# a1q123456/image_stitching

Measured on AMD Instinct MI355X. Metric: 4K frames stitched/sec, higher is better.
Workload: dtype u8

## Files before the change

### image_stitching_amd/csrc/orb.hip

```cpp
#include "common.h"
#include "dev_math.h"
#include <algorithm>
#include <cmath>
#include <mutex>
#include <unordered_map>

#define ORB_MAX_LEVELS 16
#define ORB_BORDER 32

namespace {

struct LevelDesc {
    int w, h;
    int pp;
    int sp;
    size_t pad_off;
    size_t map_off;
    float scale;
    int nfeat;
    int n2;
    int tiles_x, tiles_y, tile_off;
    int cap1, cand_off;
    int cap2, fin_off;
    int tab_off;
};

struct Levels {
    int n;
    int fast_t, patch, half_patch, edge;
    LevelDesc d[ORB_MAX_LEVELS];
};

struct Work {
    uint8_t *pad, *blur, *score, *nms;
    int* hist;
    int* thr;
    int* tile_cnt;
    uint32_t* surv_xy;
    uint8_t* surv_sc;
    int* cnt1;
    int* cnt2;
    int* flags;
    uint32_t* cand_xy;
    float* cand_resp;
    uint32_t* fin_xy;
    float* fin_resp;
    int* tab;
    int* umax;
    int8_t* pattern;
};

constexpr int ORB_BATCH = 16;
struct OrbIO {
    const uint8_t* src[ORB_BATCH];
    size_t sstride[ORB_BATCH];
    int aligned[ORB_BATCH];
    MisKeyPoint* kps[ORB_BATCH];
    uint32_t* lxy[ORB_BATCH];
    int* n_dev[ORB_BATCH];
    uint8_t* desc[ORB_BATCH];
};
#define WS_OFF(p, f, ws) p = (decltype(p))((const char*)(p) + (size_t)(f) * (ws))

constexpr int GRAY_ROWS = 4;
__global__ __launch_bounds__(256) void gray_kernel(OrbIO io, int w, int h, uint8_t* dst, int pp, size_t ws) {
    const int x = (blockIdx.x * 256 + threadIdx.x) * 4, y0 = blockIdx.y * GRAY_ROWS, f = blockIdx.z;
    if (x >= w) return;
    const uint8_t* bgr = io.src[f];
    const size_t stride = io.sstride[f];
    const int aligned = io.aligned[f];
    WS_OFF(dst, f, ws);
    const int nrows = min(GRAY_ROWS, h - y0);
    if (aligned && x + 4 <= w) {
        unsigned w0[GRAY_ROWS], w1[GRAY_ROWS], w2[GRAY_ROWS];
#pragma unroll
        for (int r = 0; r < GRAY_ROWS; r++) {
            const unsigned* sp = reinterpret_cast<const unsigned*>(bgr + (size_t)min(y0 + r, h - 1) * stride + 3 * (size_t)x);
            w0[r] = sp[0]; w1[r] = sp[1]; w2[r] = sp[2];
        }
#pragma unroll
        for (int r = 0; r < GRAY_ROWS; r++) {
            if (r >= nrows) break;
            const unsigned g0 = ((w0[r] & 255) * 3735 + ((w0[r] >> 8) & 255) * 19235 + ((w0[r] >> 16) & 255) * 9798 + (1 << 14)) >> 15;
            const unsigned g1 = ((w0[r] >> 24) * 3735 + (w1[r] & 255) * 19235 + ((w1[r] >> 8) & 255) * 9798 + (1 << 14)) >> 15;
            const unsigned g2 = (((w1[r] >> 16) & 255) * 3735 + (w1[r] >> 24) * 19235 + (w2[r] & 255) * 9798 + (1 << 14)) >> 15;
            const unsigned g3 = (((w2[r] >> 8) & 255) * 3735 + ((w2[r] >> 16) & 255) * 19235 + (w2[r] >> 24) * 9798 + (1 << 14)) >> 15;
            *reinterpret_cast<unsigned*>(dst + (size_t)(y0 + r + ORB_BORDER) * pp + ORB_BORDER + x) = g0 | (g1 << 8) | (g2 << 16) | (g3 << 24);
        }
    } else {
        for (int r = 0; r < nrows; r++) {
            const uint8_t* s = bgr + (size_t)(y0 + r) * stride + 3 * (size_t)x;
            uint8_t* o = dst + (size_t)(y0 + r + ORB_BORDER) * pp + ORB_BORDER + x;
            for (int k = 0; k < 4 && x + k < w; k++) o[k] = (uint8_t)((s[3 * k] * 3735 + s[3 * k + 1] * 19235 + s[3 * k + 2] * 9798 + (1 << 14)) >> 15);
        }
    }
}

__device__ __forceinline__ unsigned byte_at(unsigned w0, unsigned w1, unsigned w2, int o) {
    const unsigned long long lo = (unsigned long long)w0 | ((unsigned long long)w1 << 32);
    return (o < 8 ? (unsigned)(lo >> (8 * o)) : (w2 >> (8 * (o - 8)))) & 255u;
}
#ifndef MIS_RS_ROWS
#define MIS_RS_ROWS 4
#endif
constexpr int RS_ROWS = MIS_RS_ROWS;
__global__ __launch_bounds__(256) void resize_kernel(const uint8_t* __restrict__ src, int sw, int sh, int spp, uint8_t* __restrict__ dst, int dw, int dh, int dpp,
                                                     const int* __restrict__ tab, size_t ws) {
    const int x = (blockIdx.x * 64 + (threadIdx.x & 63)) * 4;
    const int ybase = __builtin_amdgcn_readfirstlane((blockIdx.y * 4 + (threadIdx.x >> 6)) * RS_ROWS);
    if (x >= dw || ybase >= dh) return;
    WS_OFF(src, blockIdx.z, ws); WS_OFF(dst, blockIdx.z, ws);
    const int dw4 = (dw + 3) & ~3;
    const int *xo = tab, *xm = tab + dw4, *yo = tab + 2 * dw4, *ym = tab + 2 * dw4 + dh;
    const int4 o4 = *reinterpret_cast<const int4*>(xo + x), m4 = *reinterpret_cast<const int4*>(xm + x);
    const int xs[4] = {o4.x, o4.y, o4.z, o4.w}, ms[4] = {m4.x, m4.y, m4.z, m4.w};
    const int nvalid = min(4, dw - x), nrows = min(RS_ROWS, dh - ybase);
    const int base = xs[0] & ~3, last = xs[nvalid - 1] + 1 - base;
    const uint8_t* r0[RS_ROWS];
    const uint8_t* r1[RS_ROWS];
    int my1[RS_ROWS];
#pragma unroll
    for (int r = 0; r < RS_ROWS; r++) {
        const int y = min(ybase + r, dh - 1);
        const int y0 = yo[y], y1 = y0 + 1 < sh ? y0 + 1 : y0;
        my1[r] = ym[y];
        r0[r] = src + (size_t)(y0 + ORB_BORDER) * spp + ORB_BORDER;
        r1[r] = src + (size_t)(y1 + ORB_BORDER) * spp + ORB_BORDER;
    }
    uint8_t* out = dst + (size_t)(ybase + ORB_BORDER) * dpp + ORB_BORDER + x;
    unsigned res[RS_ROWS];
    if (last <= 11) {
        unsigned a[RS_ROWS][3], b[RS_ROWS][3];
#pragma unroll
        for (int r = 0; r < RS_ROWS; r++) {
            const unsigned* p0 = reinterpret_cast<const unsigned*>(r0[r] + base);
            const unsigned* p1 = reinterpret_cast<const unsigned*>(r1[r] + base);
            a[r][0] = p0[0]; a[r][1] = p0[1]; a[r][2] = p0[2]; b[r][0] = p1[0]; b[r][1] = p1[1]; b[r][2] = p1[2];
        }
#pragma unroll
        for (int r = 0; r < RS_ROWS; r++) res[r] = 0;
#pragma unroll
        for (int k = 0; k < 4; k++) {
            const int o = xs[k] - base, mx1 = ms[k], mx0 = 256 - mx1;
            const bool ok = k < nvalid;
            const int oo = ok ? o : 0;
            const bool p1 = oo >= 4, p2 = oo >= 8;
#pragma unroll
            for (int r = 0; r < RS_ROWS; r++) {
                const unsigned alo = p2 ? a[r][2] : (p1 ? a[r][1] : a[r][0]), ahi = p2 ? 0u : (p1 ? a[r][2] : a[r][1]);
                const unsigned blo = p2 ? b[r][2] : (p1 ? b[r][1] : b[r][0]), bhi = p2 ? 0u : (p1 ? b[r][2] : b[r][1]);
                const unsigned ta = __builtin_amdgcn_alignbyte(ahi, alo, (unsigned)oo & 3u), tb = __builtin_amdgcn_alignbyte(bhi, blo, (unsigned)oo & 3u);
                const unsigned h0 = (ta & 255u) * mx0 + ((ta >> 8) & 255u) * mx1;
                const unsigned h1 = (tb & 255u) * mx0 + ((tb >> 8) & 255u) * mx1;
                res[r] |= ok ? ((h0 * (256 - my1[r]) + h1 * my1[r] + (1u << 15)) >> 16) << (8 * k) : 0u;
            }
        }
    } else {
#pragma unroll
        for (int r = 0; r < RS_ROWS; r++) {
            res[r] = 0;
#pragma unroll
            for (int k = 0; k < 4; k++) {
                if (k >= nvalid) break;
                const int x0 = xs[k], x1 = x0 + 1 < sw ? x0 + 1 : x0, mx1 = ms[k], mx0 = 256 - mx1;
                const unsigned h0 = (unsigned)r0[r][x0] * mx0 + (unsigned)r0[r][x1] * mx1;
                const unsigned h1 = (unsigned)r1[r][x0] * mx0 + (unsigned)r1[r][x1] * mx1;
                res[r] |= ((h0 * (256 - my1[r]) + h1 * my1[r] + (1u << 15)) >> 16) << (8 * k);
            }
        }
    }
#pragma unroll
    for (int r = 0; r < RS_ROWS; r++) {
        if (r >= nrows) break;
        uint8_t* o = out + (size_t)r * dpp;
        if (nvalid == 4) *reinterpret_cast<unsigned*>(o) = res[r];
        else
            for (int k = 0; k < nvalid; k++) o[k] = (uint8_t)(res[r] >> (8 * k));
    }
}

template <bool SIDES>
__global__ __launch_bounds__(256) void border_kernel(Levels L, uint8_t* pad, size_t ws) {
    const int f = blockIdx.z / L.n;
    const LevelDesc& d = L.d[blockIdx.z - f * L.n];
    WS_OFF(pad, f, ws);
    const int B = ORB_BORDER, pw = d.w + 2 * B, ph = d.h + 2 * B;
    uint8_t* p = pad + d.pad_off;
    if (!SIDES) {
        const int px4 = (blockIdx.x * 256 + threadIdx.x) * 4;
        if (px4 >= pw) return;
        const bool inner = px4 >= B && px4 + 3 < B + d.w;
        unsigned v[4];
        size_t drow[4], srow[4];
#pragma unroll
        for (int r = 0; r < 4; r++) {
            const int yy = blockIdx.y * 4 + r, py = yy < B ? yy : ph - 2 * B + yy;
            srow[r] = (size_t)(mis_reflect101(py - B, d.h) + B) * d.pp; drow[r] = (size_t)py * d.pp;
        }
        if (inner) {
#pragma unroll
            for (int r = 0; r < 4; r++) v[r] = *reinterpret_cast<const unsigned*>(p + srow[r] + px4);
#pragma unroll
            for (int r = 0; r < 4; r++) *reinterpret_cast<unsigned*>(p + drow[r] + px4) = v[r];
        } else {
#pragma unroll
            for (int r = 0; r < 4; r++)
                for (int k = 0; k < 4 && px4 + k < pw; k++) p[drow[r] + px4 + k] = p[srow[r] + mis_reflect101(px4 + k - B, d.w) + B];
        }
        return;
    }
    const int t = blockIdx.x * 256 + threadIdx.x, row = t >> 4, g = t & 15;
    if (row >= d.h) return;
    const int px = g < 8 ? 4 * g : pw - B + 4 * (g - 8);
    const size_t ro = (size_t)(row + B) * d.pp;
    unsigned v = 0;
#pragma unroll
    for (int k = 0; k < 4; k++) v |= (unsigned)p[ro + mis_reflect101(px + k - B, d.w) + B] << (8 * k);
    if ((px & 3) == 0) *reinterpret_cast<unsigned*>(p + ro + px) = v;
    else
#pragma unroll
        for (int k = 0; k < 4; k++) p[ro + px + k] = (uint8_t)(v >> (8 * k));
}

__device__ __forceinline__ bool fast_pretest(const uint8_t* p, int pp, int t) {
    const int v = p[0], hi = v + t, lo = v - t;
    const int c0 = p[3 * pp], c4 = p[3], c8 = p[-3 * pp], c12 = p[-3];
    unsigned br = (c0 > hi) | ((c4 > hi) << 2) | ((c8 > hi) << 4) | ((c12 > hi) << 6);
    unsigned dk = (c0 < lo) | ((c4 < lo) << 2) | ((c8 < lo) << 4) | ((c12 < lo) << 6);
    const unsigned adj_b = br & ((br >> 2) | (br << 6)), adj_d = dk & ((dk >> 2) | (dk << 6));
    if (!((adj_b | adj_d) & 0x55)) return false;
    const int c2 = p[2 * pp + 2], c6 = p[-2 * pp + 2], c10 = p[-2 * pp - 2], c14 = p[2 * pp - 2];
    br |= ((c2 > hi) << 1) | ((c6 > hi) << 3) | ((c10 > hi) << 5) | ((c14 > hi) << 7);
    dk |= ((c2 < lo) << 1) | ((c6 < lo) << 3) | ((c10 < lo) << 5) | ((c14 < lo) << 7);
    const unsigned b2 = br | (br << 8), d2 = dk | (dk << 8);
    const unsigned rb = b2 & (b2 >> 1) & (b2 >> 2) & (b2 >> 3), rd = d2 & (d2 >> 1) & (d2 >> 2) & (d2 >> 3);
    return ((rb | rd) & 0xff) != 0;
}
__device__ __forceinline__ int fast_score_full(const uint8_t* p, int pp, int t) {
    const int v = p[0];
    int d[16];
    d[0] = v - p[3 * pp]; d[1] = v - p[3 * pp + 1]; d[2] = v - p[2 * pp + 2]; d[3] = v - p[pp + 3];
    d[4] = v - p[3]; d[5] = v - p[-pp + 3]; d[6] = v - p[-2 * pp + 2]; d[7] = v - p[-3 * pp + 1];
    d[8] = v - p[-3 * pp]; d[9] = v - p[-3 * pp - 1]; d[10] = v - p[-2 * pp - 2]; d[11] = v - p[-pp - 3];
    d[12] = v - p[-3]; d[13] = v - p[pp - 3]; d[14] = v - p[2 * pp - 2]; d[15] = v - p[3 * pp - 1];
    int n3[16], x3[16];
#pragma unroll
    for (int i = 0; i < 16; i++) {
        n3[i] = min(min(d[i], d[(i + 1) & 15]), d[(i + 2) & 15]);
        x3[i] = max(max(d[i], d[(i + 1) & 15]), d[(i + 2) & 15]);
    }
    int A = -512, Bm = 512;
#pragma unroll
    for (int i = 0; i < 16; i++) {
        A = max(A, min(min(n3[i], n3[(i + 3) & 15]), n3[(i + 6) & 15]));
        Bm = min(Bm, max(max(x3[i], x3[(i + 3) & 15]), x3[(i + 6) & 15]));
    }
    const int best = max(A, -Bm);
    return best > t ? best - 1 : 0;
}
__device__ __forceinline__ int fast_score_px(const uint8_t* p, int pp, int t) { return fast_pretest(p, pp, t) ? fast_score_full(p, pp, t) : 0; }

#ifndef MIS_FT_ROWS
#define MIS_FT_ROWS 64
#endif
constexpr int FT_COLS = 64, FT_ROWS = MIS_FT_ROWS, FG_PITCH = 96, FG_COL0 = 15, HIST_COPIES = 8;
constexpr int FT_WR = (FT_ROWS + 2 + 3) / 4;
constexpr int FT_SLOTS = FT_COLS * FT_ROWS / 4;
#ifdef MIS_ORB_STATS
__device__ unsigned long long g_orb_stats[8];
#endif
__global__ __launch_bounds__(256) void fast_nms_kernel(Levels L, const uint8_t* pad, int* hist, int* tile_cnt, uint32_t* surv_xy, uint8_t* surv_sc, size_t ws) {
    __shared__ __attribute__((aligned(16))) uint8_t g[(FT_ROWS + 10) * FG_PITCH];
    __shared__ __attribute__((aligned(16))) uint8_t sc[(FT_ROWS + 2) * (FT_COLS + 4)];
    __shared__ int lh[256];
    __shared__ int lcount;
    __shared__ uint32_t lxy[FT_SLOTS];
    __shared__ uint8_t lsc[FT_SLOTS];
    __shared__ unsigned short queue[(FT_ROWS + 2) * (FT_COLS + 2)];
    __shared__ int qcount;
    const int fz = blockIdx.z / L.n, lz = blockIdx.z - fz * L.n;
    const LevelDesc& d = L.d[lz];
    const int x0 = blockIdx.x * FT_COLS, y0 = blockIdx.y * FT_ROWS, t = threadIdx.x;
    if (x0 >= d.w || y0 >= d.h) return;
    WS_OFF(pad, fz, ws); WS_OFF(hist, fz, ws); WS_OFF(tile_cnt, fz, ws); WS_OFF(surv_xy, fz, ws); WS_OFF(surv_sc, fz, ws);
    lh[t] = 0;
    if (t == 0) { lcount = 0; qcount = 0; }
    {
        const int ph = d.h + 2 * ORB_BORDER;
        const uint8_t* src = pad + d.pad_off;
        const int px0 = x0 - 16 + ORB_BORDER, py0 = y0 - 4 + ORB_BORDER;
        for (int i = t; i < (FT_ROWS + 8) * (FG_PITCH / 16); i += 256) {
            const int r = i / (FG_PITCH / 16), c = i - r * (FG_PITCH / 16);
            const int py = min(py0 + r, ph - 1);
            int px = px0 + 16 * c;
            if (px + 15 >= d.pp) px = d.pp - 16;
            reinterpret_cast<uint4*>(g)[i] = *reinterpret_cast<const uint4*>(src + (size_t)py * d.pp + px);
        }
    }
    __syncthreads();
    const int SP = FT_COLS + 4;
    for (int i = t; i < (FT_ROWS + 2) * SP / 4; i += 256) reinterpret_cast<unsigned*>(sc)[i] = 0u;
    {
        const int wv = __builtin_amdgcn_readfirstlane(t >> 6), lane = t & 63;
        const unsigned ft = (unsigned)L.fast_t;
        const int r0 = FT_WR * wv;
        bool pass[FT_WR + 1];
        unsigned long long ball[FT_WR + 1];
        int total = 0;
        {
            const uint8_t* colp = g + r0 * FG_PITCH + (lane + FG_COL0);
            unsigned col[FT_WR + 6];
#pragma unroll
            for (int j = 0; j < FT_WR + 6; j++) col[j] = colp[j * FG_PITCH];
            const int x = x0 - 1 + lane;
            const bool xin = x >= 3 && x < d.w - 3;
            const uint8_t* rowp = g + (r0 + 3) * FG_PITCH + (lane + FG_COL0 - 3);
#pragma unroll
            for (int k = 0; k < FT_WR; k++) {
                const int r = r0 + k, y = y0 - 1 + r;
                const bool rowok = r < FT_ROWS + 2 && y >= 3 && y < d.h - 3;
                const unsigned v = col[k + 3];
                const unsigned dv = max(__builtin_amdgcn_sad_u8(col[k + 6], v, 0u), __builtin_amdgcn_sad_u8(col[k], v, 0u));
                const unsigned dh = max(__builtin_amdgcn_sad_u8(rowp[k * FG_PITCH + 6], v, 0u), __builtin_amdgcn_sad_u8(rowp[k * FG_PITCH], v, 0u));
                pass[k] = rowok & xin & (min(dv, dh) > ft);
                ball[k] = __ballot(pass[k]);
                total += __popcll(ball[k]);
            }
        }
        {
            const int k = lane >> 1, cc = FT_COLS + (lane & 1), r = r0 + k, y = y0 - 1 + r, x = x0 - 1 + cc;
            bool ps = false;
            if (lane < 2 * FT_WR && r < FT_ROWS + 2) {
                const uint8_t* pp = g + (r + 3) * FG_PITCH + (cc + FG_COL0);
                const unsigned v = pp[0];
                const unsigned dv = max(__builtin_amdgcn_sad_u8(pp[3 * FG_PITCH], v, 0u), __builtin_amdgcn_sad_u8(pp[-3 * FG_PITCH], v, 0u));
                const unsigned dh = max(__builtin_amdgcn_sad_u8(pp[3], v, 0u), __builtin_amdgcn_sad_u8(pp[-3], v, 0u));
                ps = x >= 3 && x < d.w - 3 && y >= 3 && y < d.h - 3 && min(dv, dh) > ft;
            }
            pass[FT_WR] = ps;
            ball[FT_WR] = __ballot(ps);
            total += __popcll(ball[FT_WR]);
        }
        int base = 0;
        if (lane == 0 && total) base = atomicAdd(&qcount, total);
        base = __builtin_amdgcn_readfirstlane(base);
        const unsigned long long below = (1ull << lane) - 1ull;
#pragma unroll
        for (int k = 0; k < FT_WR + 1; k++) {
            if (pass[k]) {
                const int r = k < FT_WR ? r0 + k : r0 + (lane >> 1), c = k < FT_WR ? lane : FT_COLS + (lane & 1);
                queue[base + __popcll(ball[k] & below)] = (unsigned short)(r * (FT_COLS + 2) + c);
            }
            base += __popcll(ball[k]);
        }
    }
    __syncthreads();
    for (int q = t; q < qcount; q += 256) {
        const int i = queue[q], r = i / (FT_COLS + 2), c = i - r * (FT_COLS + 2);
        const int fsv = fast_score_full(g + (r + 3) * FG_PITCH + (c + FG_COL0), FG_PITCH, L.fast_t);
        sc[r * SP + c] = (uint8_t)fsv;
#ifdef MIS_ORB_STATS
        if (fsv) atomicAdd(&g_orb_stats[3], 1ull);
#endif
    }
    __syncthreads();
    {
        const int nq = qcount;
        for (int q0 = 0; q0 < nq; q0 += 256) {
            const int q = q0 + t;
            bool keep = false;
// ... 280 lines not shown
        for (int k = 0; k < ORB_MAX_LEVELS; k++) c[k] = k < L.n ? cnt2[min(k, L.n - 1)] : 0;
#pragma unroll
        for (int k = 0; k < ORB_MAX_LEVELS; k++) {
            if (j >= total + c[k]) { base = total + c[k]; l = k + 1; }
            total += c[k];
        }
    }
    if (blockIdx.x == 0 && threadIdx.x == 0) *n_out = min(total, cap_out);
    if (j >= total || j >= cap_out) return;
    const LevelDesc& d = L.d[l];
    const int i = j - base;
    uint32_t xy = fin_xy[d.fin_off + i];
    int x = xy & 0xffff, y = xy >> 16;
    const int pp = d.pp, hp = L.half_patch;
    const uint8_t* ctr = pad + d.pad_off + (size_t)(y + ORB_BORDER) * pp + (x + ORB_BORDER);
    int m01 = 0, m10 = 0;
    const int u = lane - hp;
    if (with_angle && lane <= 2 * hp) {
        m10 = u * ctr[u];
        if (hp <= 15) {
            int um[16], vp[16], vm[16];
#pragma unroll
            for (int v = 1; v <= 15; ++v) um[v] = umax[min(v, hp)];
#pragma unroll
            for (int v = 1; v <= 15; ++v) { const int vv = min(v, hp); vp[v] = ctr[u + vv * pp]; vm[v] = ctr[u - vv * pp]; }
#pragma unroll
            for (int v = 1; v <= 15; ++v) {
                const bool in = v <= hp && abs(u) <= um[v];
                m10 += in ? u * (vp[v] + vm[v]) : 0;
                m01 += in ? v * (vp[v] - vm[v]) : 0;
            }
        } else {
            for (int v = 1; v <= hp; ++v) {
                if (abs(u) <= umax[v]) {
                    int vp = ctr[u + v * pp], vm = ctr[u - v * pp];
                    m10 += u * (vp + vm);
                    m01 += v * (vp - vm);
                }
            }
        }
    }
#pragma unroll
    for (int o = 32; o > 0; o >>= 1) { m01 += __shfl_xor(m01, o); m10 += __shfl_xor(m10, o); }
    if (lane == 0) {
        MisKeyPoint kp;
        kp.x = (float)x * d.scale; kp.y = (float)y * d.scale;
        kp.size = (float)L.patch * d.scale;
        kp.angle = with_angle ? mis_fast_atan2((float)m01, (float)m10) : 0.f;
        kp.response = fin_resp[d.fin_off + i];
        kp.octave = l;
        kps[base + i] = kp;
        kp_lxy[base + i] = xy;
    }
}

__global__ __launch_bounds__(256) void blur_kernel(Levels L, const uint8_t* pad, uint8_t* blur) {
    constexpr int TR = 32, TP = 80;
    __shared__ __attribute__((aligned(16))) uint8_t tile[(TR + 6) * TP];
    __shared__ __attribute__((aligned(16))) uint16_t hbuf[(TR + 6) * 64];
    const LevelDesc& d = L.d[blockIdx.z];
    const int pw = d.w + 2 * ORB_BORDER, ph = d.h + 2 * ORB_BORDER;
    const int tx0 = blockIdx.x * 64, ty0 = blockIdx.y * TR, t = threadIdx.x;
    if (tx0 >= pw || ty0 >= ph) return;
    const uint8_t* src = pad + d.pad_off;
    uint8_t* dst = blur + d.pad_off;
    for (int i = t; i < (TR + 6) * (TP / 4); i += 256) {
        const int r = i / (TP / 4), c = i - r * (TP / 4);
        const int sy = min(max(ty0 + r - 3, 0), ph - 1);
        int sx = tx0 - 4 + 4 * c;
        sx = min(max(sx, 0), d.pp - 4);
        reinterpret_cast<unsigned*>(tile)[i] = *reinterpret_cast<const unsigned*>(src + (size_t)sy * d.pp + sx);
    }
    __syncthreads();
    const int kq[7] = {18, 34, 48, 56, 48, 34, 18};
    for (int i = t; i < (TR + 6) * 16; i += 256) {
        const int r = i >> 4, cg = i & 15;
        const unsigned* p = reinterpret_cast<const unsigned*>(tile + r * TP + 4 * cg);
        const unsigned w0 = p[0], w1 = p[1], w2 = p[2];
        int b[12];
#pragma unroll
        for (int k = 0; k < 4; k++) { b[k] = (w0 >> (8 * k)) & 255; b[4 + k] = (w1 >> (8 * k)) & 255; b[8 + k] = (w2 >> (8 * k)) & 255; }
        unsigned short o[4];
#pragma unroll
        for (int k = 0; k < 4; k++) {
            int acc = 0;
#pragma unroll
            for (int j = 0; j < 7; j++) acc += kq[j] * b[k + 1 + j];
            o[k] = (unsigned short)acc;
        }
        *reinterpret_cast<uint2*>(hbuf + r * 64 + 4 * cg) = make_uint2(o[0] | ((unsigned)o[1] << 16), o[2] | ((unsigned)o[3] << 16));
    }
    __syncthreads();
    const int c = t & 63, px = tx0 + c;
    if (px >= pw) return;
    const int r0 = (t >> 6) * (TR / 4);
    int hv[TR / 4 + 6];
#pragma unroll
    for (int j = 0; j < TR / 4 + 6; j++) hv[j] = hbuf[(r0 + j) * 64 + c];
#pragma unroll
    for (int k = 0; k < TR / 4; k++) {
        const int r = r0 + k, py = ty0 + r;
        if (py >= ph) break;
        const int x = px - ORB_BORDER, y = py - ORB_BORDER;
        uint8_t o;
        if ((unsigned)x < (unsigned)d.w && (unsigned)y < (unsigned)d.h) {
            int acc = 0;
#pragma unroll
            for (int j = 0; j < 7; j++) acc += kq[j] * hv[k + j];
            o = (uint8_t)((acc + (1 << 15)) >> 16);
        } else o = tile[(r + 3) * TP + c + 4];
        dst[(size_t)py * d.pp + px] = o;
    }
}

__global__ __launch_bounds__(256) void describe_kernel(Levels L, const uint8_t* blur, const MisKeyPoint* kps, const uint32_t* kp_lxy,
                                                       const int* n_ptr, const int8_t* pattern, uint8_t* desc) {
    const int i = blockIdx.x * 8 + (threadIdx.x >> 5), b = threadIdx.x & 31;
    if (i >= *n_ptr) return;
    const MisKeyPoint kp = kps[i];
    const LevelDesc& d = L.d[kp.octave];
    const float inv = 1.f / d.scale;
    const int cx = mis_round_f(kp.x * inv), cy = mis_round_f(kp.y * inv);
    float ang = kp.angle * (float)(3.14159265358979323846 / 180.f);
    float sa, ca;
    mis_sincosf(ang, &sa, &ca);
    const int pp = d.pp;
    const uint8_t* ctr = blur + d.pad_off + (size_t)(cy + ORB_BORDER) * pp + (cx + ORB_BORDER);
    const int8_t* pat = pattern + b * 32;
    int val = 0;
#pragma unroll
    for (int bit = 0; bit < 8; bit++) {
        float x0 = (float)pat[4 * bit], y0 = (float)pat[4 * bit + 1], x1 = (float)pat[4 * bit + 2], y1 = (float)pat[4 * bit + 3];
        int ix0 = mis_round_f(x0 * ca - y0 * sa), iy0 = mis_round_f(x0 * sa + y0 * ca);
        int ix1 = mis_round_f(x1 * ca - y1 * sa), iy1 = mis_round_f(x1 * sa + y1 * ca);
        int t0 = ctr[iy0 * pp + ix0], t1 = ctr[iy1 * pp + ix1];
        val |= (t0 < t1) << bit;
    }
    desc[(size_t)i * 32 + b] = (uint8_t)val;
}

constexpr int DD_R = 28, DD_P = DD_R + 3, DD_N = 2 * DD_P + 1, DD_ROW_DW = (DD_N + 3 + 3) / 4, DD_PITCH = 4 * DD_ROW_DW + 4;
struct UMax16 { int v[16]; };
__global__ __launch_bounds__(256) void describe_direct_kernel(Levels L, const uint8_t* pad, OrbIO io, const int8_t* pattern, const int* umax, UMax16 um16, size_t ws) {
    __shared__ __attribute__((aligned(16))) uint8_t patch[4][DD_N * DD_PITCH];
    const int wave = threadIdx.x >> 6, lane = threadIdx.x & 63;
    const int i = blockIdx.x * 4 + wave, fr = blockIdx.y;
    WS_OFF(pad, fr, ws);
    MisKeyPoint* kps = io.kps[fr];
    const uint32_t* kp_lxy = io.lxy[fr];
    const int* n_ptr = io.n_dev[fr];
    uint8_t* desc = io.desc[fr];
    if (i >= *n_ptr) return;
    const MisKeyPoint kp = kps[i];
    const LevelDesc& d = L.d[kp.octave];
    const float inv = 1.f / d.scale;
    const int cx = mis_round_f(kp.x * inv), cy = mis_round_f(kp.y * inv);
    const int pp = d.pp;
    const uint8_t* org = pad + d.pad_off + (size_t)(cy + ORB_BORDER - DD_P) * pp + (cx + ORB_BORDER - DD_P);
    const int shift = (int)((uintptr_t)org & 3);
    const uint8_t* abase = org - shift;
    uint8_t* P = patch[wave];
    for (int k = lane; k < DD_N * DD_ROW_DW; k += 64) {
        const int r = k / DD_ROW_DW, c = k - r * DD_ROW_DW;
        reinterpret_cast<unsigned*>(P + r * DD_PITCH)[c] = *reinterpret_cast<const unsigned*>(abase + (size_t)r * pp + 4 * c);
    }
    __builtin_amdgcn_fence(__ATOMIC_ACQ_REL, "wavefront");
    __builtin_amdgcn_wave_barrier();
    const int c0 = DD_P * DD_PITCH + DD_P + shift;
    float kp_angle;
    {
        const int hp = L.half_patch;
        const uint8_t* ctr = P + c0;
        int m01 = 0, m10 = 0;
        const int u = lane - hp;
        if (lane <= 2 * hp) {
            m10 = u * ctr[u];
            if (hp <= 15) {
#pragma unroll 3
                for (int v = 1; v <= hp; ++v) {
                    const int vp = ctr[u + v * DD_PITCH], vm = ctr[u - v * DD_PITCH];
                    const bool in = abs(u) <= um16.v[v];
                    m10 += in ? u * (vp + vm) : 0;
                    m01 += in ? v * (vp - vm) : 0;
                }
            } else {
                for (int v = 1; v <= hp; ++v) {
                    if (abs(u) <= umax[v]) {
                        const int vp = ctr[u + v * DD_PITCH], vm = ctr[u - v * DD_PITCH];
                        m10 += u * (vp + vm);
                        m01 += v * (vp - vm);
                    }
                }
            }
        }
#pragma unroll
        for (int o = 32; o > 0; o >>= 1) { m01 += __shfl_xor(m01, o); m10 += __shfl_xor(m10, o); }
        kp_angle = mis_fast_atan2((float)m01, (float)m10);
        if (lane == 0) kps[i].angle = kp_angle;
    }
    float ang = kp_angle * (float)(3.14159265358979323846 / 180.f);
    float sa, ca;
    mis_sincosf(ang, &sa, &ca);
    const int b = lane & 31, h = lane >> 5;
    const int8_t* pat = pattern + b * 32 + h * 16;
    const unsigned* P32 = reinterpret_cast<const unsigned*>(P);
    auto blurred = [&](int ix, int iy) {
        const int a = c0 + (iy - 3) * DD_PITCH + (ix - 3);
        const bool inside = (unsigned)(cx + ix) < (unsigned)d.w && (unsigned)(cy + iy) < (unsigned)d.h;
        const unsigned* q = P32 + (a >> 2);
        const unsigned sh = (unsigned)(a & 3) << 3;
        const int kq[7] = {18, 34, 48, 56, 48, 34, 18};
        unsigned acc = 0, centre = 0;
#pragma unroll
        for (int j = 0; j < 7; j++) {
            const unsigned d0 = q[j * (DD_PITCH / 4)], d1 = q[j * (DD_PITCH / 4) + 1], d2 = q[j * (DD_PITCH / 4) + 2];
            const unsigned lo = __builtin_amdgcn_alignbit(d1, d0, sh), hi = __builtin_amdgcn_alignbit(d2, d1, sh);
            const unsigned hs = __builtin_amdgcn_udot4(lo, 0x38302212u, __builtin_amdgcn_udot4(hi, 0x00122230u, 0u, false), false);
            acc += (unsigned)kq[j] * hs;
            if (j == 3) centre = lo >> 24;
        }
        return inside ? (int)((acc + (1u << 15)) >> 16) : (int)centre;
    };
    int val = 0;
#ifndef DD_UNROLL
#define DD_UNROLL 1
#endif
#pragma unroll DD_UNROLL
    for (int bit = 0; bit < 4; bit++) {
        float x0 = (float)pat[4 * bit], y0 = (float)pat[4 * bit + 1], x1 = (float)pat[4 * bit + 2], y1 = (float)pat[4 * bit + 3];
        int ix0 = mis_round_f(x0 * ca - y0 * sa), iy0 = mis_round_f(x0 * sa + y0 * ca);
        int ix1 = mis_round_f(x1 * ca - y1 * sa), iy1 = mis_round_f(x1 * sa + y1 * ca);
        const int t0 = blurred(ix0, iy0), t1 = blurred(ix1, iy1);
        val |= (t0 < t1) << (bit + 4 * h);
    }
    val |= __shfl_xor(val, 32);
    if (h == 0) desc[(size_t)i * 32 + b] = (uint8_t)val;
}

constexpr int ORB_GATHER_MAX = 96;
struct GatherPtrs { const int* p[ORB_GATHER_MAX]; };
__global__ void gather_ints_kernel(GatherPtrs g, int n, int* __restrict__ out) {
    const int i = blockIdx.x * blockDim.x + threadIdx.x;
    if (i < n) out[i] = *g.p[i];
}

}

struct MisOrb {
    MisContext* ctx = nullptr;
    void (*enqueued_cb)(void*) = nullptr;
    void* enqueued_user = nullptr;
    MisOrbParams p;
    int max_w = 0, max_h = 0;
    int cur_w = 0, cur_h = 0;
    Levels L;
    Work w;
    size_t ws_stride = 0;
    int ws_frames = 0;
    int umax_host[64] = {0};
    int8_t pattern_host[1024] = {0};
    void* mem = nullptr;
    size_t pad_bytes = 0, map_bytes = 0;
    int cand_total = 0, fin_total = 0, tab_total = 0, surv_total = 0, out_cap = 0;
    std::vector<int> tab_host;
    int* host_counts = nullptr;
    bool direct_describe = false;
};

namespace {

void linear_exact_coeffs(int dlen, int slen, int* ofs, int* m1) {
    double inv = (double)dlen / (double)slen, scale = 1.0 / inv;
    for (int i = 0; i < dlen; i++) {
        double v = ((double)i + 0.5) * scale - 0.5;
        int iv = (int)floor(v);
        if (iv < 0) { ofs[i] = 0; m1[i] = 0; }
        else if (iv >= slen - 1) { ofs[i] = slen - 1; m1[i] = 0; }
        else { ofs[i] = iv; m1[i] = (int)lrint((v - (double)iv) * 256.0); }
    }
}

constexpr int ORB_MAX_LEVEL_FEATURES = 2048 - 128;

inline float level_scale(const MisOrbParams& p, int l) { return (float)pow((double)p.scale_factor, (double)l); }
inline int level_dim(int len, float sc) { return (int)lrint((double)((float)len / sc)); }

void level_budgets(const MisOrbParams& p, int* nfeat) {
    float factor = (float)(1.0 / (double)p.scale_factor);
    float nd = (float)p.nfeatures * (1 - factor) / (1 - (float)pow((double)factor, (double)p.nlevels));
    int sum = 0;
    for (int l = 0; l < p.nlevels - 1; l++) { nfeat[l] = (int)lrintf(nd); sum += nfeat[l]; nd *= factor; }
    nfeat[p.nlevels - 1] = std::max(p.nfeatures - sum, 0);
}

int check_level_sizes(MisContext* ctx, const MisOrbParams& p, int w, int h) {
    for (int l = 0; l < p.nlevels; l++) {
        const float sc = level_scale(p, l);
        MIS_CHECK(ctx, level_dim(w, sc) >= 1 && level_dim(h, sc) >= 1, MIS_E_UNSUPPORTED,
                  "ORB level %d of a %dx%d frame is empty (scale_factor %g, nlevels %d)", l, w, h, (double)p.scale_factor, p.nlevels);
    }
    return MIS_OK;
}

void plan_levels(MisOrb* o, int w, int h) {
    Levels& L = o->L;
    const MisOrbParams& p = o->p;
    L.n = p.nlevels; L.fast_t = p.fast_threshold; L.patch = p.patch_size; L.half_patch = p.patch_size / 2; L.edge = p.edge_threshold;
    size_t pad_off = 0, map_off = 0;
    int cand_off = 0, fin_off = 0, tab_off = 0, surv_off = 0;
    int nfeat[ORB_MAX_LEVELS];
    level_budgets(p, nfeat);
    for (int l = 0; l < L.n; l++) {
        LevelDesc& d = L.d[l];
        float sc = level_scale(p, l);
        d.scale = sc;
        d.w = level_dim(w, sc);
        d.h = level_dim(h, sc);
        d.pp = (int)mis_align_up((size_t)d.w + 2 * ORB_BORDER, 64);
        d.sp = (int)mis_align_up((size_t)d.w, 64);
        d.pad_off = pad_off; pad_off += (size_t)d.pp * (d.h + 2 * ORB_BORDER);
        d.map_off = map_off; map_off += (size_t)d.sp * d.h;
        d.nfeat = nfeat[l];
        d.n2 = p.score_type == 0 ? 2 * d.nfeat : d.nfeat;
        d.tiles_x = (d.w + FT_COLS - 1) / FT_COLS; d.tiles_y = (d.h + FT_ROWS - 1) / FT_ROWS;
        d.tile_off = surv_off; surv_off += d.tiles_x * d.tiles_y;
        d.cap1 = 4 * d.n2 + 4096;
        d.cap2 = std::min(d.nfeat + 128, 2048);
        d.cand_off = cand_off; cand_off += d.cap1;
        d.fin_off = fin_off; fin_off += d.cap2;
        d.tab_off = tab_off; tab_off += (2 * ((d.w + 3) & ~3) + 2 * d.h + 3) & ~3;
    }
    o->pad_bytes = pad_off; o->map_bytes = map_off; o->cand_total = cand_off; o->fin_total = fin_off; o->tab_total = tab_off; o->surv_total = surv_off;
    o->tab_host.assign(tab_off, 0);
    for (int l = 1; l < L.n; l++) {
        int* t = o->tab_host.data() + L.d[l].tab_off;
        const int dw4 = (L.d[l].w + 3) & ~3;
        linear_exact_coeffs(L.d[l].w, L.d[l - 1].w, t, t + dw4);
        linear_exact_coeffs(L.d[l].h, L.d[l - 1].h, t + 2 * dw4, t + 2 * dw4 + L.d[l].h);
    }
}

int upload_tables(MisOrb* o) {
    MisContext* ctx = o->ctx;
    if (o->tab_total)
        MIS_HIP(ctx, hipMemcpyAsync(o->w.tab, o->tab_host.data(), sizeof(int) * o->tab_total, hipMemcpyHostToDevice, ctx->stream));
    MIS_HIP(ctx, hipStreamSynchronize(ctx->stream));
    return MIS_OK;
}

std::mutex g_feat_mutex;
std::unordered_map<void*, size_t> g_feat_sizes;

int alloc_features(MisContext* ctx, int cap, int desc_cols, int desc_dtype, MisFeatures* f) {
    size_t kb = mis_align_up(sizeof(MisKeyPoint) * (size_t)cap, 256), db = mis_align_up((size_t)cap * desc_cols * mis_dtype_size(desc_dtype), 256);
    size_t lb = mis_align_up(sizeof(uint32_t) * (size_t)cap, 256);
    void* mem = nullptr;
    size_t got = 0;
    int rc = mis_pool_alloc(ctx, kb + db + lb + 256, &mem, &got);
    if (rc != MIS_OK) return rc;
    f->keypoints = (MisKeyPoint*)mem;
    f->descriptors = (uint8_t*)mem + kb;
    f->desc_cols = desc_cols; f->desc_dtype = desc_dtype;
    f->owner_ = mem;
    f->n = 0;
    std::lock_guard<std::mutex> lock(g_feat_mutex);
    g_feat_sizes[mem] = got;
    return MIS_OK;
}

inline uint32_t* feat_lxy(const MisFeatures* f, int cap) {
    size_t kb = mis_align_up(sizeof(MisKeyPoint) * (size_t)cap, 256), db = mis_align_up((size_t)cap * f->desc_cols * mis_dtype_size(f->desc_dtype), 256);
    return (uint32_t*)((uint8_t*)f->owner_ + kb + db);
}
inline int* feat_count(const MisFeatures* f, int cap) {
    size_t kb = mis_align_up(sizeof(MisKeyPoint) * (size_t)cap, 256), db = mis_align_up((size_t)cap * f->desc_cols * mis_dtype_size(f->desc_dtype), 256);
    size_t lb = mis_align_up(sizeof(uint32_t) * (size_t)cap, 256);
    return (int*)((uint8_t*)f->owner_ + kb + db + lb);
}

int enqueue_detect_group(MisOrb* o, const DevView* img, int w, int h, MisFeatures* out, int ng) {
    MisContext* ctx = o->ctx;
    const Levels& L = o->L;
// ... 373 lines not shown
```

Before: 3463.

## Use udot2/perm in resize, cheaper reflect in border, preload ORB pattern

Rewrites the bilinear resize fast path to pack pixel pairs with byte permutes and compute weights with udot2 dot products, replacing per-pixel selects and multiplies. Adds a single-fold reflect101 for border padding when the level is larger than the border. Loads the ORB pattern as one vector load, hoisted before the patch copy, and makes the octave index wave-uniform. Together these cut ALU work in several ORB kernels. The resize fast path now applies only when the source span is at most 6 bytes, so more cases may fall back to the slow path.

Result: no change. 3433 (-0.9%).

```diff
diff --git a/image_stitching_amd/csrc/orb.hip b/image_stitching_amd/csrc/orb.hip
--- a/image_stitching_amd/csrc/orb.hip
+++ b/image_stitching_amd/csrc/orb.hip
@@ -96,9 +96,9 @@
     }
 }
 
-__device__ __forceinline__ unsigned byte_at(unsigned w0, unsigned w1, unsigned w2, int o) {
-    const unsigned long long lo = (unsigned long long)w0 | ((unsigned long long)w1 << 32);
-    return (o < 8 ? (unsigned)(lo >> (8 * o)) : (w2 >> (8 * (o - 8)))) & 255u;
+__device__ __forceinline__ unsigned udot2_u16(unsigned a, unsigned b, unsigned c) {
+    typedef unsigned short us2 __attribute__((ext_vector_type(2)));
+    return __builtin_amdgcn_udot2(__builtin_bit_cast(us2, a), __builtin_bit_cast(us2, b), c, false);
 }
 #ifndef MIS_RS_ROWS
 #define MIS_RS_ROWS 4
@@ -115,21 +115,26 @@
     const int4 o4 = *reinterpret_cast<const int4*>(xo + x), m4 = *reinterpret_cast<const int4*>(xm + x);
     const int xs[4] = {o4.x, o4.y, o4.z, o4.w}, ms[4] = {m4.x, m4.y, m4.z, m4.w};
     const int nvalid = min(4, dw - x), nrows = min(RS_ROWS, dh - ybase);
-    const int base = xs[0] & ~3, last = xs[nvalid - 1] + 1 - base;
+    const int xlast = nvalid == 4 ? xs[3] : (nvalid == 3 ? xs[2] : (nvalid == 2 ? xs[1] : xs[0]));
     const uint8_t* r0[RS_ROWS];
     const uint8_t* r1[RS_ROWS];
-    int my1[RS_ROWS];
+    unsigned my1[RS_ROWS];
+    int ys[RS_ROWS];
 #pragma unroll
     for (int r = 0; r < RS_ROWS; r++) {
         const int y = min(ybase + r, dh - 1);
-        const int y0 = yo[y], y1 = y0 + 1 < sh ? y0 + 1 : y0;
-        my1[r] = ym[y];
+        ys[r] = yo[y]; my1[r] = (unsigned)ym[y];
+    }
+#pragma unroll
+    for (int r = 0; r < RS_ROWS; r++) {
+        const int y0 = ys[r], y1 = y0 + 1 < sh ? y0 + 1 : y0;
         r0[r] = src + (size_t)(y0 + ORB_BORDER) * spp + ORB_BORDER;
         r1[r] = src + (size_t)(y1 + ORB_BORDER) * spp + ORB_BORDER;
     }
     uint8_t* out = dst + (size_t)(ybase + ORB_BORDER) * dpp + ORB_BORDER + x;
     unsigned res[RS_ROWS];
-    if (last <= 11) {
+    if (xlast - xs[0] <= 6) {
+        const unsigned base = (unsigned)xs[0] & ~3u, shf = (unsigned)xs[0] & 3u;
         unsigned a[RS_ROWS][3], b[RS_ROWS][3];
 #pragma unroll
         for (int r = 0; r < RS_ROWS; r++) {
@@ -137,23 +142,26 @@
             const unsigned* p1 = reinterpret_cast<const unsigned*>(r1[r] + base);
             a[r][0] = p0[0]; a[r][1] = p0[1]; a[r][2] = p0[2]; b[r][0] = p1[0]; b[r][1] = p1[1]; b[r][2] = p1[2];
         }
-#pragma unroll
-        for (int r = 0; r < RS_ROWS; r++) res[r] = 0;
+        unsigned sel[4], wx[4];
 #pragma unroll
         for (int k = 0; k < 4; k++) {
-            const int o = xs[k] - base, mx1 = ms[k], mx0 = 256 - mx1;
-            const bool ok = k < nvalid;
-            const int oo = ok ? o : 0;
-            const bool p1 = oo >= 4, p2 = oo >= 8;
-#pragma unroll
-            for (int r = 0; r < RS_ROWS; r++) {
-                const unsigned alo = p2 ? a[r][2] : (p1 ? a[r][1] : a[r][0]), ahi = p2 ? 0u : (p1 ? a[r][2] : a[r][1]);
-                const unsigned blo = p2 ? b[r][2] : (p1 ? b[r][1] : b[r][0]), bhi = p2 ? 0u : (p1 ? b[r][2] : b[r][1]);
-                const unsigned ta = __builtin_amdgcn_alignbyte(ahi, alo, (unsigned)oo & 3u), tb = __builtin_amdgcn_alignbyte(bhi, blo, (unsigned)oo & 3u);
-                const unsigned h0 = (ta & 255u) * mx0 + ((ta >> 8) & 255u) * mx1;
-                const unsigned h1 = (tb & 255u) * mx0 + ((tb >> 8) & 255u) * mx1;
-                res[r] |= ok ? ((h0 * (256 - my1[r]) + h1 * my1[r] + (1u << 15)) >> 16) << (8 * k) : 0u;
+            const unsigned o = k < nvalid ? (unsigned)(xs[k] - xs[0]) : 0u;
+            sel[k] = 0x0c010c00u + (o | (o << 16));
+            wx[k] = (256u - (unsigned)ms[k]) | ((unsigned)ms[k] << 16);
+        }
+#pragma unroll
+        for (int r = 0; r < RS_ROWS; r++) {
+            const unsigned a0 = __builtin_amdgcn_alignbyte(a[r][1], a[r][0], shf), a1 = __builtin_amdgcn_alignbyte(a[r][2], a[r][1], shf);
+            const unsigned b0 = __builtin_amdgcn_alignbyte(b[r][1], b[r][0], shf), b1 = __builtin_amdgcn_alignbyte(b[r][2], b[r][1], shf);
+            const unsigned wy = (256u - my1[r]) | (my1[r] << 16);
+            unsigned v[4];
+#pragma unroll
+            for (int k = 0; k < 4; k++) {
+                const unsigned h0 = udot2_u16(__builtin_amdgcn_perm(a1, a0, sel[k]), wx[k], 0u);
+                const unsigned h1 = udot2_u16(__builtin_amdgcn_perm(b1, b0, sel[k]), wx[k], 0u);
+                v[k] = udot2_u16(h0 | (h1 << 16), wy, 1u << 15);
             }
+            res[r] = __builtin_amdgcn_perm(__builtin_amdgcn_perm(v[3], v[2], 0x0c0c0602u), __builtin_amdgcn_perm(v[1], v[0], 0x0c0c0602u), 0x05040100u);
         }
     } else {
 #pragma unroll
@@ -179,6 +187,12 @@
     }
 }
 
+__device__ __forceinline__ int ring_reflect101(int p, int len, bool one_fold) {
+    if (!one_fold) return mis_reflect101(p, len);
+    const int q = p < 0 ? -p : p;
+    return q >= len ? 2 * len - 2 - q : q;
+}
+
 template <bool SIDES>
 __global__ __launch_bounds__(256) void border_kernel(Levels L, uint8_t* pad, size_t ws) {
     const int f = blockIdx.z / L.n;
@@ -186,6 +200,7 @@
     WS_OFF(pad, f, ws);
     const int B = ORB_BORDER, pw = d.w + 2 * B, ph = d.h + 2 * B;
     uint8_t* p = pad + d.pad_off;
+    const bool fold_x = d.w > B, fold_y = d.h > B;
     if (!SIDES) {
         const int px4 = (blockIdx.x * 256 + threadIdx.x) * 4;
         if (px4 >= pw) return;
@@ -195,7 +210,7 @@
 #pragma unroll
         for (int r = 0; r < 4; r++) {
             const int yy = blockIdx.y * 4 + r, py = yy < B ? yy : ph - 2 * B + yy;
-            srow[r] = (size_t)(mis_reflect101(py - B, d.h) + B) * d.pp; drow[r] = (size_t)py * d.pp;
+            srow[r] = (size_t)(ring_reflect101(py - B, d.h, fold_y) + B) * d.pp; drow[r] = (size_t)py * d.pp;
         }
         if (inner) {
 #pragma unroll
@@ -205,7 +220,7 @@
         } else {
 #pragma unroll
             for (int r = 0; r < 4; r++)
-                for (int k = 0; k < 4 && px4 + k < pw; k++) p[drow[r] + px4 + k] = p[srow[r] + mis_reflect101(px4 + k - B, d.w) + B];
+                for (int k = 0; k < 4 && px4 + k < pw; k++) p[drow[r] + px4 + k] = p[srow[r] + ring_reflect101(px4 + k - B, d.w, fold_x) + B];
         }
         return;
     }
@@ -215,7 +230,7 @@
     const size_t ro = (size_t)(row + B) * d.pp;
     unsigned v = 0;
 #pragma unroll
-    for (int k = 0; k < 4; k++) v |= (unsigned)p[ro + mis_reflect101(px + k - B, d.w) + B] << (8 * k);
+    for (int k = 0; k < 4; k++) v |= (unsigned)p[ro + ring_reflect101(px + k - B, d.w, fold_x) + B] << (8 * k);
     if ((px & 3) == 0) *reinterpret_cast<unsigned*>(p + ro + px) = v;
     else
 #pragma unroll
@@ -802,10 +817,12 @@
     uint8_t* desc = io.desc[fr];
     if (i >= *n_ptr) return;
     const MisKeyPoint kp = kps[i];
-    const LevelDesc& d = L.d[kp.octave];
+    const int b = lane & 31, h = lane >> 5;
+    uint4 pat4 = *reinterpret_cast<const uint4*>(pattern + b * 32 + h * 16);
+    const LevelDesc& d = L.d[__builtin_amdgcn_readfirstlane(kp.octave)];
     const float inv = 1.f / d.scale;
     const int cx = mis_round_f(kp.x * inv), cy = mis_round_f(kp.y * inv);
-    const int pp = d.pp;
+    const int pp = d.pp, lw = d.w, lh = d.h;
     const uint8_t* org = pad + d.pad_off + (size_t)(cy + ORB_BORDER - DD_P) * pp + (cx + ORB_BORDER - DD_P);
     const int shift = (int)((uintptr_t)org & 3);
     const uint8_t* abase = org - shift;
@@ -851,12 +868,10 @@
     float ang = kp_angle * (float)(3.14159265358979323846 / 180.f);
     float sa, ca;
     mis_sincosf(ang, &sa, &ca);
-    const int b = lane & 31, h = lane >> 5;
-    const int8_t* pat = pattern + b * 32 + h * 16;
     const unsigned* P32 = reinterpret_cast<const unsigned*>(P);
     auto blurred = [&](int ix, int iy) {
         const int a = c0 + (iy - 3) * DD_PITCH + (ix - 3);
-        const bool inside = (unsigned)(cx + ix) < (unsigned)d.w && (unsigned)(cy + iy) < (unsigned)d.h;
+        const bool inside = (unsigned)(cx + ix) < (unsigned)lw && (unsigned)(cy + iy) < (unsigned)lh;
         const unsigned* q = P32 + (a >> 2);
         const unsigned sh = (unsigned)(a & 3) << 3;
         const int kq[7] = {18, 34, 48, 56, 48, 34, 18};
@@ -877,7 +892,9 @@
 #endif
 #pragma unroll DD_UNROLL
     for (int bit = 0; bit < 4; bit++) {
-        float x0 = (float)pat[4 * bit], y0 = (float)pat[4 * bit + 1], x1 = (float)pat[4 * bit + 2], y1 = (float)pat[4 * bit + 3];
+        const unsigned pw = pat4.x;
+        pat4.x = pat4.y; pat4.y = pat4.z; pat4.z = pat4.w;
+        float x0 = (float)(int8_t)pw, y0 = (float)(int8_t)(pw >> 8), x1 = (float)(int8_t)(pw >> 16), y1 = (float)(int8_t)(pw >> 24);
         int ix0 = mis_round_f(x0 * ca - y0 * sa), iy0 = mis_round_f(x0 * sa + y0 * ca);
         int ix1 = mis_round_f(x1 * ca - y1 * sa), iy1 = mis_round_f(x1 * sa + y1 * ca);
         const int t0 = blurred(ix0, iy0), t1 = blurred(ix1, iy1);
```
